# lab4d-org/lab4d

Hardware: AMD Instinct MI355X
Metric: rendered rays/sec (fwd+bwd) at 512² × 128 samples; PSNR vs ref (higher is better)
Workload: dtype bf16

## Files before the change

include/lab4d_skin.h:

```cpp
#ifndef LAB4D_SKIN_H
#define LAB4D_SKIN_H

int lab4d_bone_coords_forward(const float* xyz, const float* art_r, const float* art_d, const float* gauss, int S,
                              int spf, int M, int B, float* xyz_bone, void* stream);
int lab4d_bone_coords_backward(const float* xyz, const float* art_r, const float* art_d, const float* gauss,
                               const float* g_bone, int S, int spf, int M, int B, float* g_xyz, float* g_art_r,
                               float* g_art_d, float* g_gauss, void* stream);

int lab4d_bone_coords_backward_gram(const float* xyz, const float* art_r, const float* gauss, const float* g_bone, int S, int spf, int M, int B,
                                    float* g_xyz, float* G, void* stream);

int lab4d_bone_params_from_gram(const float* art_r, const float* art_d, const float* gauss, const float* G, int M, int B,
                                float* g_art_r, float* g_art_d, float* g_gauss, void* stream);

int lab4d_skin_blend_forward(const float* xyz, const float* art_r, const float* art_d, const float* gauss,
                             const float* delta_raw, const float* se3_r, const float* se3_d, int S, int spf, int M, int B,
                             float* out, float* entropy, float* dskin, float* work, void* stream);
int lab4d_skin_blend_backward(const float* xyz, const float* art_r, const float* art_d, const float* gauss,
                              const float* delta_raw, const float* se3_r, const float* se3_d, const float* g_out,
                              const float* g_ent, const float* g_dskin, int S, int spf, int M, int B, float* g_xyz,
                              float* g_raw, float* g_se3, float* g_art_r, float* g_art_d, float* g_gauss, float* work,
                              void* stream);
int lab4d_skin_blend_backward_acc(const float* xyz, const float* art_r, const float* art_d, const float* gauss,
                                  const float* delta_raw, const float* se3_r, const float* se3_d, const float* g_out,
                                  const float* g_ent, const float* g_dskin, int S, int spf, int M, int B, float* g_xyz,
                                  float* g_raw, float* g_se3, float* g_art_r, float* g_art_d, float* g_gauss, float* work,
                                  int accumulate, void* stream);

long long lab4d_skin_blend_backward_workspace_floats(int S, int spf, int M, int B, int has_g_se3);

int lab4d_gauss_density_forward(const float* xyz, const float* centres, int B, const float* ibeta, int S, float* out,
                                int* best, void* stream);
int lab4d_gauss_density_backward(const float* xyz, const float* centres, int B, const float* ibeta, const int* best,
                                 const float* g, int S, float* g_xyz, float* g_centres, float* g_ibeta, void* stream);

int lab4d_gram_per_frame(const float* A, int CA, const float* Bm, int CB, int S, int spf, int M, float* out, void* stream);

int lab4d_bone_affine(const float* art_r, const float* art_d, const float* gauss, int M, int B, float* aff, void* stream);

#endif
```

lab4d_amd/csrc/skinning.hip:

```cpp
#include "common.hpp"

namespace lab4d {

struct V3 { float x, y, z; };
__device__ __forceinline__ V3 operator+(V3 a, V3 b) { return {a.x + b.x, a.y + b.y, a.z + b.z}; }
__device__ __forceinline__ V3 operator-(V3 a, V3 b) { return {a.x - b.x, a.y - b.y, a.z - b.z}; }
__device__ __forceinline__ V3 operator*(V3 a, float s) { return {a.x * s, a.y * s, a.z * s}; }
__device__ __forceinline__ float dot(V3 a, V3 b) { return a.x * b.x + a.y * b.y + a.z * b.z; }
__device__ __forceinline__ V3 cross(V3 a, V3 b) { return {a.y * b.z - a.z * b.y, a.z * b.x - a.x * b.z, a.x * b.y - a.y * b.x}; }
__device__ __forceinline__ V3 ldv3(const float* p) { return {p[0], p[1], p[2]}; }
__device__ __forceinline__ void stv3(float* p, V3 v) { p[0] = v.x; p[1] = v.y; p[2] = v.z; }

__device__ __forceinline__ V3 qrot(float w, V3 v, V3 p) { return p * (w * w - dot(v, v)) + v * (2.f * dot(v, p)) + cross(v, p) * (2.f * w); }
__device__ __forceinline__ V3 qrot_t(float w, V3 v, V3 g) { return g * (w * w - dot(v, v)) + v * (2.f * dot(v, g)) - cross(v, g) * (2.f * w); }
__device__ __forceinline__ void qrot_gq(float w, V3 v, V3 p, V3 g, float& gw, V3& gv) {
  const float gp = dot(g, p), gvv = dot(g, v), vp = dot(v, p);
  gw = 2.f * w * gp + 2.f * dot(g, cross(v, p));
  gv = v * (-2.f * gp) + p * (2.f * gvv) + g * (2.f * vp) + cross(p, g) * (2.f * w);
}


template <int C>
struct RowTile {
  static constexpr int CP = C | 1;
// ... 490 lines not shown
        const float gskin = bl.p[b_] * (gp[b_] - pg) + ge * (bl.p[b_] - (b_ == bl.anchor ? 1.f : 0.f));
        const float gsk = -2.f * gskin;
        const Aff A = ld_aff(affm + 12 * b_);
        const V3 c = bone_coord(A, x);
        const float u0 = gsk * c.x, u1 = gsk * c.y, u2 = gsk * c.z;
        gx = gx + V3{A.r0.x * u0 + A.r1.x * u1 + A.r2.x * u2, A.r0.y * u0 + A.r1.y * u1 + A.r2.y * u2, A.r0.z * u0 + A.r1.z * u1 + A.r2.z * u2};
      }
      if (accumulate) gx = gx + ldv3(g_xyz + s * 3);
      stv3(g_xyz + s * 3, gx);
      if (!FUSE) {
        float* xx = work + S * (2 * B + 8) + s * 10;
        xx[0] = x.x * x.x; xx[1] = x.x * x.y; xx[2] = x.x * x.z; xx[3] = x.x;
        xx[4] = x.y * x.y; xx[5] = x.y * x.z; xx[6] = x.y;
        xx[7] = x.z * x.z; xx[8] = x.z; xx[9] = 1.f;
      }
    }
    __syncthreads();
    if (active) {
#pragma unroll
      for (int b_ = 0; b_ < B; ++b_) row[b_] = bl.p[b_] * bl.sg[b_];
    }
    __syncthreads();
    if (FUSE) gram(n, 8, 0);
    else { T::store(work, s0, n, tile); __syncthreads(); }
    if (active) {
#pragma unroll
      for (int b_ = 0; b_ < B; ++b_) {
        const float gskin = bl.p[b_] * (gp[b_] - pg) + ge * (bl.p[b_] - (b_ == bl.anchor ? 1.f : 0.f));
        row[b_] = -2.f * gskin;
      }
      if (FUSE) {
        float* xx = aux + threadIdx.x * AUXW;
        xx[0] = x.x * x.x; xx[1] = x.x * x.y; xx[2] = x.x * x.z; xx[3] = x.x;
        xx[4] = x.y * x.y; xx[5] = x.y * x.z; xx[6] = x.y;
        xx[7] = x.z * x.z; xx[8] = x.z; xx[9] = 1.f;
      }
    }
    __syncthreads();
    if (FUSE) gram(n, 10, B * 8);
    else { T::store(work + S * (B + 8), s0, n, tile); __syncthreads(); }
    if (active) {
#pragma unroll
      for (int b_ = 0; b_ < B; ++b_) {
        const float gskin = bl.p[b_] * (gp[b_] - pg) + ge * (bl.p[b_] - (b_ == bl.anchor ? 1.f : 0.f));
        const float gdelta = -gskin + gds * bl.dl[b_];
        row[b_] = ((rawpos >> b_) & 1u) ? 0.1f * gdelta : 0.f;
      }
    }
    __syncthreads();
    T::store(g_raw, s0, n, tile, accumulate);
    __syncthreads();
  }
  if (FUSE && cur_m >= 0) flush(cur_m);
}

__global__ void __launch_bounds__(64) k_bone_gram_from_moments(const float* __restrict__ ar, const float* __restrict__ ad,
                                                                const float* __restrict__ gauss, const float* __restrict__ Q, int M, int B,
                                                                float* __restrict__ G) {
  const int i = blockIdx.x * blockDim.x + threadIdx.x;
  if (i >= M * B) return;
  const int b = i % B;
  const float* r = ar + (size_t)i * 4;
  const float* d = ad + (size_t)i * 4;
  const float w = r[0], dw = d[0];
  const V3 v = ldv3(r + 1), dv = ldv3(d + 1), gs = ldv3(gauss + 3 * b);
  const V3 e0 = {1.f, 0.f, 0.f}, e1 = {0.f, 1.f, 0.f}, e2 = {0.f, 0.f, 1.f};
  const V3 t = (v * dw - dv * w + cross(v, dv)) * 2.f;
  const V3 c0 = qrot(w, v * -1.f, e0), c1 = qrot(w, v * -1.f, e1), c2 = qrot(w, v * -1.f, e2);
  const float A[3][4] = {{c0.x, c1.x, c2.x, t.x}, {c0.y, c1.y, c2.y, t.y}, {c0.z, c1.z, c2.z, t.z}};
  const float* q = Q + (size_t)i * 10;
  const float Qm[4][4] = {{q[0], q[1], q[2], q[3]}, {q[1], q[4], q[5], q[6]}, {q[2], q[5], q[7], q[8]}, {q[3], q[6], q[8], q[9]}};
  const float ig[3] = {1.f / gs.x, 1.f / gs.y, 1.f / gs.z};
  float* o = G + (size_t)i * 12;
#pragma unroll
  for (int k = 0; k < 3; ++k)
#pragma unroll
    for (int j = 0; j < 4; ++j) o[4 * k + j] = ig[k] * (A[k][0] * Qm[0][j] + A[k][1] * Qm[1][j] + A[k][2] * Qm[2][j] + A[k][3] * Qm[3][j]);
}

__global__ void __launch_bounds__(640) k_gram_pf(const float* __restrict__ A, int CA, const float* __restrict__ Bm, int CB, long S, int spf,
                                                  int chunk, float* __restrict__ out) {
  constexpr int TS = 128;
  extern __shared__ float sm[];
  float* sa = sm;
  float* sb = sm + TS * CA;
  const int m = blockIdx.y;
  const long f0 = (long)m * spf, f1 = min(S, f0 + spf);
  const long c0 = f0 + (long)blockIdx.x * chunk, c1 = min(f1, c0 + chunk);
  if (c0 >= c1) return;
  const int t = threadIdx.x;
  const int i = t / CB, j = t - i * CB;
  const bool active = t < CA * CB;
  float acc = 0.f;
  for (long s0 = c0; s0 < c1; s0 += TS) {
    const int n = (int)min((long)TS, c1 - s0);
    for (int e = t; e < n * CA; e += blockDim.x) sa[e] = A[s0 * CA + e];
    for (int e = t; e < n * CB; e += blockDim.x) sb[e] = Bm[s0 * CB + e];
    __syncthreads();
    if (active)
      for (int k = 0; k < n; ++k) acc += sa[k * CA + i] * sb[k * CB + j];
    __syncthreads();
  }
  if (active) atomicAdd(out + ((size_t)m * CA + i) * CB + j, acc);
}

template <int CB>
// ... 140 lines not shown
                                         const float* sr, const float* sd, const float* g_out, const float* g_ent, const float* g_dskin, int S,
                                         int spf, int M, int B, float* g_xyz, float* g_raw, float* g_se3, float* g_art_r, float* g_art_d,
                                         float* g_gauss, float* work, void* stream) {
  return lab4d_skin_blend_backward_acc(xyz, art_r, art_d, gauss, raw, sr, sd, g_out, g_ent, g_dskin, S, spf, M, B, g_xyz, g_raw, g_se3, g_art_r, g_art_d,
                                       g_gauss, work, 0, stream);
}
extern "C" int lab4d_skin_blend_backward_acc(const float* xyz, const float* art_r, const float* art_d, const float* gauss, const float* raw,
                                             const float* sr, const float* sd, const float* g_out, const float* g_ent, const float* g_dskin, int S,
                                             int spf, int M, int B, float* g_xyz, float* g_raw, float* g_se3, float* g_art_r, float* g_art_d,
                                             float* g_gauss, float* work, int accumulate, void* stream) {
  LAB4D_REQUIRE(xyz && art_r && art_d && gauss && raw && sr && sd && g_out && g_xyz && g_raw && work, "skin_blend_backward: null pointer");
  LAB4D_REQUIRE(spf > 0 && (long)M * spf >= S, "skin_blend_backward: M*spf < S");
  SKIN_REQUIRE_BONES(B);
  if (S == 0) return LAB4D_OK;
  hipStream_t st = (hipStream_t)stream;
  float* aff = work;
  float* Q = work + (size_t)M * B * 12;
  float* G = Q + (size_t)M * B * 10;
  float* ws = G + (size_t)M * B * 12;
  const bool fused = blend_bwd_fused(spf, g_se3 != nullptr);
  const bool params = g_art_r || g_art_d || g_gauss;
  hipLaunchKernelGGL(k_bone_affine, dim3(div_up(M * B, 64)), dim3(64), 0, st, art_r, art_d, gauss, M, B, aff);
  if (fused || params)
    if (int e = zero_async(Q, (size_t)M * B * 10 * sizeof(float), st)) return e;
  if (fused) {
    const int grid = grid_1d(S, 256, 2048);
#define BLEND_BWD(UNI_, FUSE_, GRID_)                                                                                                              \
  do {                                                                                                                                              \
    if (accumulate) { SKIN_DISPATCH(B, hipLaunchKernelGGL((k_blend_bwd<NB, UNI_, FUSE_, true>), dim3(GRID_), dim3(256), 0, st, xyz, aff, raw, sr, sd, g_out, \
                                                          g_ent, g_dskin, (long)S, spf, g_xyz, g_raw, ws, g_se3, Q)); }                              \
    else { SKIN_DISPATCH(B, hipLaunchKernelGGL((k_blend_bwd<NB, UNI_, FUSE_, false>), dim3(GRID_), dim3(256), 0, st, xyz, aff, raw, sr, sd, g_out,       \
                                               g_ent, g_dskin, (long)S, spf, g_xyz, g_raw, ws, g_se3, Q)); }                                         \
  } while (0)
    BLEND_BWD(true, true, grid);
  } else if (spf % 256 == 0) {
    BLEND_BWD(true, false, grid_1d(S, 256, 8192));
  } else {
    BLEND_BWD(false, false, grid_1d(S, 256, 8192));
  }
#undef BLEND_BWD
  if (int e = check_launch("skin_blend_backward")) return e;
  if (g_se3 && !fused)
    if (int e = lab4d_gram_per_frame(ws, B, ws + (size_t)S * B, 8, S, spf, M, g_se3, stream)) return e;
  if (params) {
    if (!fused)
      if (int e = lab4d_gram_per_frame(ws + (size_t)S * (B + 8), B, ws + (size_t)S * (2 * B + 8), 10, S, spf, M, Q, stream)) return e;
    hipLaunchKernelGGL(k_bone_gram_from_moments, dim3(div_up(M * B, 64)), dim3(64), 0, st, art_r, art_d, gauss, Q, M, B, G);
    if (int e = check_launch("bone_gram_from_moments")) return e;
    return lab4d_bone_params_from_gram(art_r, art_d, gauss, G, M, B, g_art_r, g_art_d, g_gauss, stream);
  }
  return LAB4D_OK;
}

namespace lab4d {
__global__ void __launch_bounds__(256) k_gauss_density_fwd(const float* __restrict__ xyz, const float* __restrict__ centres, int B,
                                                            const float* __restrict__ ibeta_p, long S, float* __restrict__ out, int* __restrict__ best) {
  const float ibeta = *ibeta_p;
  for (long s = (long)blockIdx.x * blockDim.x + threadIdx.x; s < S; s += (long)gridDim.x * blockDim.x) {
    const V3 x = ldv3(xyz + s * 3);
    float dmin = INFINITY;
    int bi = 0;
    for (int b = 0; b < B; ++b) {
      const V3 d = x - ldv3(centres + 3 * b);
      const float d2 = dot(d, d);
      if (d2 < dmin) { dmin = d2; bi = b; }
    }
    out[s] = expf(-0.5f * (dmin / (0.01f * 0.01f))) * ibeta;
    if (best) best[s] = bi;
  }
}
__global__ void __launch_bounds__(256) k_gauss_density_bwd(const float* __restrict__ xyz, const float* __restrict__ centres, int B,
                                                            const float* __restrict__ ibeta_p, const int* __restrict__ best, const float* __restrict__ g, long S,
                                                            float* __restrict__ g_xyz, float* __restrict__ g_centres, float* __restrict__ g_ibeta) {
  extern __shared__ float acc[];
  const float ibeta = *ibeta_p;
  for (int i = threadIdx.x; i < 3 * B + 1; i += blockDim.x) acc[i] = 0.f;
  __syncthreads();
  for (long s = (long)blockIdx.x * blockDim.x + threadIdx.x; s < S; s += (long)gridDim.x * blockDim.x) {
    const int b = best[s];
    const V3 d = ldv3(xyz + s * 3) - ldv3(centres + 3 * b);
    const float e = expf(-0.5f * (dot(d, d) / (0.01f * 0.01f)));
    const float gs = g[s];
    const V3 gx = d * (-gs * e * ibeta / (0.01f * 0.01f));
    if (g_xyz) stv3(g_xyz + s * 3, gx);
    atomicAdd(&acc[3 * b + 0], -gx.x); atomicAdd(&acc[3 * b + 1], -gx.y); atomicAdd(&acc[3 * b + 2], -gx.z);
    atomicAdd(&acc[3 * B], gs * e);
  }
  __syncthreads();
  for (int i = threadIdx.x; i < 3 * B; i += blockDim.x) if (acc[i] != 0.f) atomicAdd(g_centres + i, acc[i]);
  if (threadIdx.x == 0 && g_ibeta) atomicAdd(g_ibeta, acc[3 * B]);
}
}

extern "C" int lab4d_gauss_density_forward(const float* xyz, const float* centres, int B, const float* ibeta, int S, float* out, int* best, void* stream) {
  LAB4D_REQUIRE(xyz && centres && out && ibeta, "gauss_density_forward: null pointer");
  if (S == 0) return LAB4D_OK;
  hipLaunchKernelGGL(lab4d::k_gauss_density_fwd, dim3(grid_1d(S, 256, 8192)), dim3(256), 0, (hipStream_t)stream, xyz, centres, B, ibeta, (long)S, out, best);
  return check_launch("gauss_density_forward");
}
extern "C" int lab4d_gauss_density_backward(const float* xyz, const float* centres, int B, const float* ibeta, const int* best, const float* g, int S,
                                            float* g_xyz, float* g_centres, float* g_ibeta, void* stream) {
  LAB4D_REQUIRE(xyz && centres && ibeta && best && g && g_centres, "gauss_density_backward: null pointer");
  LAB4D_REQUIRE(B <= 64, "gauss_density_backward: B too large");
  if (S == 0) return LAB4D_OK;
  const int grid = grid_1d(S, 256, 1024);
  hipLaunchKernelGGL(lab4d::k_gauss_density_bwd, dim3(grid), dim3(256), (3 * B + 1) * sizeof(float), (hipStream_t)stream, xyz, centres, B, ibeta, best, g,
// ... 20 lines not shown
```

lab4d_amd/warping.py:

```python
import os

import torch
from torch.autograd import Function
from torch.autograd.function import once_differentiable

from . import _lib, mlp
from . import quat_utils as Q


def _blend_bwd_work(S, spf, M, B, device):
    n = int(_lib.lib().lab4d_skin_blend_backward_workspace_floats(S, spf, M, B, 1))
    return torch.empty(n, device=device), n == M * B * 34


FUSE_BONE_COORDS = os.environ.get("LAB4D_FUSE_BONE", "1") != "0"


class BoneCoords(Function):

    @staticmethod
    def forward(ctx, xyz, art_r, art_d, gauss, spf):
        xyz, art_r, art_d, gauss = xyz.contiguous(), art_r.contiguous(), art_d.contiguous(), gauss.contiguous()
        _lib.require_device(xyz, art_r, art_d, gauss)
        S, (M, B) = xyz.shape[0], art_r.shape[:2]
        out = torch.empty(S, 3 * B, device=xyz.device)
        with _lib.timed("k_bone_fwd", (0.0, 4.0 * S * (3 + 3 * B))):
            _lib.call("bone_coords_forward", xyz, art_r, art_d, gauss, S, spf, M, B, out)
        ctx.save_for_backward(xyz, art_r, art_d, gauss)
        ctx.spf = spf
        return out

    @staticmethod
    @once_differentiable
    def backward(ctx, g):
        return (*bone_coords_backward(ctx.saved_tensors, ctx.spf, ctx.needs_input_grad[1:4], g), None)


def bone_coords_backward(saved, spf, need, g):
    xyz, art_r, art_d, gauss = saved
    need_r, need_d, need_g = need
    S, (M, B) = xyz.shape[0], art_r.shape[:2]
    g = g.contiguous()
    gx = torch.empty_like(xyz)
    if any(need) and spf % 256 == 0 and os.environ.get("LAB4D_BONE_FUSE", "1") != "0":
        G = torch.empty(M, 3 * B, 4, device=xyz.device)
        with _lib.timed("k_bone_bwd_x+gram", (2.0 * S * 3 * B * 4, 4.0 * S * (3 + 3 + 3 * B))):
            _lib.call("bone_coords_backward_gram", xyz, art_r, gauss, g, S, spf, M, B, gx, G)
    else:
        with _lib.timed("k_bone_bwd_x", (0.0, 4.0 * S * (3 + 3 * B))):
            _lib.call("bone_coords_backward", xyz, art_r, art_d, gauss, g, S, spf, M, B, gx, None, None, None)
        if not any(need):
            return gx, None, None, None
# ... 78 lines not shown
    def forward(ctx, net, prec, spf, xyz, tab, *params):
        want = mlp.Wants(x=any(ctx.needs_input_grad), params=ctx.needs_input_grad[SkinChainA.N_LEAD:])
        out, _, ctx.chain = mlp.chain_forward(net, prec, spf, xyz.contiguous(), (), params, want, aff=tab.detach().contiguous())
        return out

    @staticmethod
    @once_differentiable
    def backward(ctx, d_out):
        d_x, _, _, _, g_params = mlp.chain_backward(ctx.chain, d_out)
        return (None, None, None, d_x, ctx.chain.g_aff, *g_params)


SKIN_AFFINE = os.environ.get("LAB4D_SKIN_AFFINE", "1") != "0"


class SkinBlend(Function):

    @staticmethod
    def forward(ctx, xyz, raw, art_r, art_d, gauss, se3_r, se3_d, spf):
        xyz, raw, art_r, art_d, gauss, se3_r, se3_d = [t.contiguous() for t in (xyz, raw, art_r, art_d, gauss, se3_r, se3_d)]
        _lib.require_device(xyz, raw, art_r, art_d, gauss, se3_r, se3_d)
        S, (M, B) = xyz.shape[0], se3_r.shape[:2]
        out = torch.empty(S, 3, device=xyz.device)
        ent = torch.empty(S, 1, device=xyz.device)
        dsk = torch.empty(S, 1, device=xyz.device)
        work = torch.empty(M * B * 12, device=xyz.device)
        with _lib.timed("k_blend_fwd", (0.0, 4.0 * S * (3 + B + 3 + 2))):
            _lib.call("skin_blend_forward", xyz, art_r, art_d, gauss, raw, se3_r, se3_d, S, spf, M, B, out, ent, dsk, work)
        ctx.save_for_backward(xyz, raw, art_r, art_d, gauss, se3_r, se3_d)
        ctx.spf = spf
        return out, ent, dsk

    @staticmethod
    @once_differentiable
    def backward(ctx, g_out, g_ent, g_dsk):
        xyz, raw, art_r, art_d, gauss, se3_r, se3_d = ctx.saved_tensors
        S, (M, B) = xyz.shape[0], se3_r.shape[:2]
        g_out = g_out.contiguous()
        g_ent = g_ent.contiguous() if g_ent is not None else None
        g_dsk = g_dsk.contiguous() if g_dsk is not None else None
        gx, gr = torch.empty_like(xyz), torch.empty_like(raw)
        gse3 = torch.zeros(M, B, 8, device=xyz.device)
        need_p = any(ctx.needs_input_grad[2:5])
        gar = torch.empty_like(art_r) if need_p else None
        gad = torch.empty_like(art_d) if need_p else None
        gg = torch.zeros_like(gauss) if need_p else None
        work, fused = _blend_bwd_work(S, ctx.spf, M, B, xyz.device)
        with _lib.timed("k_blend_bwd+gram", (0.0, 4.0 * S * ((3 + B + 3 + 2) + (3 + B) + (0 if fused else 2 * (2 * B + 18))))):
            _lib.call("skin_blend_backward", xyz, art_r, art_d, gauss, raw, se3_r, se3_d, g_out, g_ent, g_dsk, S, ctx.spf, M, B, gx, gr, gse3, gar, gad, gg,
                      work)
        return gx, gr, gar, gad, gg, gse3[..., :4].contiguous(), gse3[..., 4:].contiguous(), None


class SkinBlendMulti(Function):

    @staticmethod
    def forward(ctx, xyz, raw, art_r, art_d, gauss, spf, *se3s):
        xyz, raw, art_r, art_d, gauss = [t.contiguous() for t in (xyz, raw, art_r, art_d, gauss)]
        se3s = [t.contiguous() for t in se3s]
        _lib.require_device(xyz, raw, art_r, art_d, gauss, *se3s)
        S, (M, B) = xyz.shape[0], art_r.shape[:2]
        outs = []
        for i in range(0, len(se3s), 2):
            out = torch.empty(S, 3, device=xyz.device)
            ent = torch.empty(S, 1, device=xyz.device)
            dsk = torch.empty(S, 1, device=xyz.device)
            work = torch.empty(M * B * 12, device=xyz.device)
            with _lib.timed("k_blend_fwd", (0.0, 4.0 * S * (3 + B + 3 + 2))):
                _lib.call("skin_blend_forward", xyz, art_r, art_d, gauss, raw, se3s[i], se3s[i + 1], S, spf, M, B, out, ent, dsk, work)
            outs += [out, ent, dsk]
        ctx.save_for_backward(xyz, raw, art_r, art_d, gauss, *se3s)
        ctx.spf = spf
        return tuple(outs)

    @staticmethod
    @once_differentiable
    def backward(ctx, *grads):
        xyz, raw, art_r, art_d, gauss, *se3s = ctx.saved_tensors
        S, (M, B) = xyz.shape[0], art_r.shape[:2]
        gx, gr = torch.empty_like(xyz), torch.empty_like(raw)
        need_p = any(ctx.needs_input_grad[2:5])
        work0, fused = _blend_bwd_work(S, ctx.spf, M, B, xyz.device)
        gar = gad = gg = None
        gse3s = []
        first = True
        for i in range(0, len(se3s), 2):
            g_out, g_ent, g_dsk = grads[3 * (i // 2):3 * (i // 2) + 3]
            if g_out is None and g_ent is None and g_dsk is None:
                gse3s += [None, None]
                continue
            g_out = torch.zeros_like(xyz) if g_out is None else g_out.contiguous()
            g_ent = g_ent.contiguous() if g_ent is not None else None
            g_dsk = g_dsk.contiguous() if g_dsk is not None else None
            gse3 = torch.zeros(M, B, 8, device=xyz.device)
            par = torch.empty_like(art_r) if need_p else None
            pad = torch.empty_like(art_d) if need_p else None
            pg = torch.zeros_like(gauss) if need_p else None
            work = work0 if first else _blend_bwd_work(S, ctx.spf, M, B, xyz.device)[0]
            with _lib.timed("k_blend_bwd+gram", (0.0, 4.0 * S * ((3 + B + 3 + 2) + (3 + B) * (1 if first else 2) + (0 if fused else 2 * (2 * B + 18))))):
                _lib.call("skin_blend_backward_acc", xyz, art_r, art_d, gauss, raw, se3s[i], se3s[i + 1], g_out, g_ent, g_dsk, S, ctx.spf, M, B, gx, gr, gse3,
                          par, pad, pg, work, 0 if first else 1)
            first = False
            if need_p:
                gar, gad, gg = (par, pad, pg) if gar is None else (gar + par, gad + pad, gg + pg)
            gse3s += [gse3[..., :4].contiguous(), gse3[..., 4:].contiguous()]
        if first:
            return (None,) * (6 + len(se3s))
        return (gx, gr, gar, gad, gg, None) + tuple(gse3s)


def get_gauss(P):
    lg = P["warp.skinning_model.log_gauss"]
    symm = P.get("warp.skinning_model.symm_idx")
    if symm is not None:
        lg = (lg[symm] + lg) / 2
    return lg.exp()


def _spf(shape):
    spf = 1
    for d in shape[1:-1]:
        spf *= d
    return spf


def skin_cond(t_embed, code, M):
    return torch.cat([t_embed.expand(M, -1), code], -1)


def skin_logits(P, x, art, t_embed, code, M, spf, prec, pre=None):
    gauss = pre["gauss"] if pre is not None else get_gauss(P)
    B = art[0].shape[1]
    net = mlp.skin_net_for(B)
    d, bd = mlp.describe(net), mlp.bindings(net, "")
    if SKIN_AFFINE and FUSE_BONE_COORDS:
        tab = pre.get("tab") if pre is not None else None
        if tab is None:
            pf = pre["pf"] if pre is not None else mlp.pf_bias_of(net, 0, P[bd[0].wname], skin_cond(t_embed, code, M))
            tab = skin_affine_table(P, art, gauss, pf, B)
        net_a = mlp.skin_net_for(B, affine=True)
        bda = mlp.bindings(net_a, "")
        params = []
        for l in range(mlp.describe(net_a).n_layers):
            params += [P[bda[l].wname], P[bda[l].bname]]
        return SkinChainA.apply(net_a, prec, spf, x, tab, *params), gauss
    pf = pre["pf"] if pre is not None else mlp.pf_bias_of(net, 0, P[bd[0].wname], skin_cond(t_embed, code, M))
    params = []
    for l in range(d.n_layers):
        params += [P[bd[l].wname], P[bd[l].bname]]
    if not FUSE_BONE_COORDS:
        bone = BoneCoords.apply(x, art[0], art[1], gauss, spf)
        return mlp.MlpChain.apply(net, prec, spf, bone, None, None, -1, 1, None, None, pf, *params), gauss
    return SkinChain.apply(net, prec, spf, x, art[0], art[1], gauss, 1, pf, *params), gauss


def skinning_warp(P, xyz, t_articulation, rest_articulation, t_embed, code, backward, prec=mlp.PREC_F32, pre=None):
    shape = xyz.shape
    M, spf = shape[0], _spf(shape)
    if pre is not None:
        se3 = pre["se3"]
        art = t_articulation if backward else rest_articulation
    elif backward:
        se3 = Q.dual_quaternion_mul(rest_articulation, Q.dual_quaternion_inverse(t_articulation))
        art = t_articulation
    else:
        se3 = Q.dual_quaternion_mul(t_articulation, Q.dual_quaternion_inverse(rest_articulation))
        art = rest_articulation
    x = xyz.reshape(-1, 3)
    raw, gauss = skin_logits(P, x, art, t_embed, code, M, spf, prec, pre)
    out, ent, dsk = SkinBlend.apply(x, raw, art[0], art[1], gauss, se3[0], se3[1], spf)
    return out.view(shape), {"skin_entropy": ent.view(shape[:-1] + (1,)), "delta_skin": dsk.view(shape[:-1] + (1,))}


def skinning_warp_forward_multi(P, xyz, t_articulations, rest_articulation, t_embed_mean, code, prec=mlp.PREC_F32, pre=None):
    shape = xyz.shape
    M, spf = shape[0], _spf(shape)
    x = xyz.reshape(-1, 3)
    raw, gauss = skin_logits(P, x, rest_articulation, t_embed_mean, code, M, spf, prec, pre)
    rest_inv = None if pre is not None else Q.dual_quaternion_inverse(rest_articulation)
    se3s = [pre["se3s"][i] if pre is not None else Q.dual_quaternion_mul(t_art, rest_inv) for i, t_art in enumerate(t_articulations)]
    flat = SkinBlendMulti.apply(x, raw, rest_articulation[0], rest_articulation[1], gauss, spf, *[t for se3 in se3s for t in se3])
    outs = []
    for i in range(len(se3s)):
        out, ent, dsk = flat[3 * i:3 * i + 3]
        outs.append((out.view(shape), {"skin_entropy": ent.view(shape[:-1] + (1,)), "delta_skin": dsk.view(shape[:-1] + (1,))}))
    return outs


def dense_warp(P, xyz, t_embed, code, backward, prec=mlp.PREC_F32, prefix="warp.post_warp.", net=mlp.NET_DENSE):
    shape = xyz.shape
    spf = 1
    for d in shape[1:-1]:
        spf *= d
    which = "backward_map." if backward else "forward_map."
    cond = torch.cat([t_embed, code], -1)
    conds = {0: cond, 4: cond} if net == mlp.NET_DENSE6 else {0: cond}
    motion = mlp.run_chain(net, prec, P, xyz.reshape(-1, 3), spf, conds=conds, prefix=prefix + which)
    return xyz + 0.1 * motion.view(shape)


def composed_warp(P, xyz, t_articulation, rest_articulation, t_embed, code, backward, prec=mlp.PREC_F32, dense=None):
    if not backward and dense is not None:
        xyz = dense_warp(P, xyz, dense["t_embed"], dense["code_fw"], False, prec)
    out, aux = skinning_warp(P, xyz, t_articulation, rest_articulation, t_embed, code, backward, prec)
    if backward and dense is not None:
        out = dense_warp(P, out, dense["t_embed"], dense["code_bw"], True, prec)
    return out, aux
```

Before: 765,400.

## Fuse two-target skin blending into single forward and backward kernels

Adds multi-target blend kernels that compute the skinning weights once per point and apply them to both target SE3 sets in one pass, in both forward and backward. The backward kernel also fuses the per-frame Gram reductions for both targets plus the bone moments, avoiding repeated launches and repeated reads of xyz and raw logits. The Python wrapper now shares the entropy and delta-skin outputs across targets and dispatches to the fused path by default when the shape matches. The fused kernels are larger and use more shared memory and registers, which may reduce occupancy.

New measurement: 775,500, median of 6. +1.3%, better.

```diff
diff --git a/include/lab4d_skin.h b/include/lab4d_skin.h
--- a/include/lab4d_skin.h
+++ b/include/lab4d_skin.h
@@ -29,6 +29,14 @@
 
 long long lab4d_skin_blend_backward_workspace_floats(int S, int spf, int M, int B, int has_g_se3);
 
+int lab4d_skin_blend_forward_multi(const float* xyz, const float* art_r, const float* art_d, const float* gauss, const float* delta_raw, int T,
+                                   const float* const* se3_r, const float* const* se3_d, int S, int spf, int M, int B, float* const* out,
+                                   float* entropy, float* dskin, float* work, void* stream);
+int lab4d_skin_blend_backward_multi(const float* xyz, const float* art_r, const float* art_d, const float* gauss, const float* delta_raw, int T,
+                                    const float* const* se3_r, const float* const* se3_d, const float* const* g_out, const float* g_ent,
+                                    const float* g_dskin, int S, int spf, int M, int B, float* g_xyz, float* g_raw, float* const* g_se3,
+                                    float* g_art_r, float* g_art_d, float* g_gauss, float* work, void* stream);
+
 int lab4d_gauss_density_forward(const float* xyz, const float* centres, int B, const float* ibeta, int S, float* out,
                                 int* best, void* stream);
 int lab4d_gauss_density_backward(const float* xyz, const float* centres, int B, const float* ibeta, const int* best,
diff --git a/lab4d_amd/csrc/skinning.hip b/lab4d_amd/csrc/skinning.hip
--- a/lab4d_amd/csrc/skinning.hip
+++ b/lab4d_amd/csrc/skinning.hip
@@ -566,6 +566,270 @@
     __syncthreads();
   }
   if (FUSE && cur_m >= 0) flush(cur_m);
+}
+
+constexpr int BLEND_GROUP = 5;
+template <int B>
+struct SkinWeights {
+  float p[B];
+  float dl[B];
+  int anchor;
+  float lse_minus_max;
+};
+template <int B>
+__device__ __forceinline__ void skin_weights(V3 x, const float* __restrict__ affm, const float* __restrict__ raw, SkinWeights<B>& o) {
+  float skin[B];
+  float mx = -INFINITY;
+  int am = 0;
+#pragma unroll
+  for (int b = 0; b < B; ++b) {
+    const V3 c = bone_coord(ld_aff(affm + 12 * b), x);
+    const float dlt = fmaxf(raw[b], 0.f) * 0.1f;
+    o.dl[b] = dlt;
+    skin[b] = -(dot(c, c) + dlt);
+    if (skin[b] > mx) { mx = skin[b]; am = b; }
+  }
+  float sum = 0.f;
+#pragma unroll
+  for (int b = 0; b < B; ++b) { o.p[b] = expf(skin[b] - mx); sum += o.p[b]; }
+  const float isum = 1.f / sum;
+  o.anchor = am;
+  o.lse_minus_max = logf(sum);
+#pragma unroll
+  for (int b = 0; b < B; ++b) o.p[b] *= isum;
+}
+template <int B>
+__device__ __forceinline__ unsigned blend_target(const SkinWeights<B>& w, const float* __restrict__ sr, const float* __restrict__ sd, float (&rw)[4],
+                                                 float (&dw4)[4], float& inv) {
+  const int am = w.anchor;
+  const float a0 = sr[4 * am], a1 = sr[4 * am + 1], a2 = sr[4 * am + 2], a3 = sr[4 * am + 3];
+  unsigned neg = 0;
+#pragma unroll
+  for (int k = 0; k < 4; ++k) { rw[k] = 0.f; dw4[k] = 0.f; }
+#pragma unroll
+  for (int b = 0; b < B; ++b) {
+    if (b % BLEND_GROUP == 0) __builtin_amdgcn_sched_barrier(0);
+    const float* r = sr + 4 * b;
+    const float* d = sd + 4 * b;
+    const bool pos = (a0 * r[0] + a1 * r[1] + a2 * r[2] + a3 * r[3]) > 0.f;
+    neg |= (pos ? 0u : 1u) << b;
+    const float c = pos ? w.p[b] : -w.p[b];
+#pragma unroll
+    for (int k = 0; k < 4; ++k) { rw[k] += c * r[k]; dw4[k] += c * d[k]; }
+  }
+  __builtin_amdgcn_sched_barrier(0);
+  inv = 1.f / sqrtf(rw[0] * rw[0] + rw[1] * rw[1] + rw[2] * rw[2] + rw[3] * rw[3]);
+  return neg;
+}
+
+template <typename P>
+__device__ __forceinline__ P pick(int t, P a0, P a1) { return t == 0 ? a0 : a1; }
+
+template <int B, int T>
+__global__ void __launch_bounds__(256) k_blend_fwd_multi(const float* __restrict__ xyz, const float* __restrict__ aff, const float* __restrict__ raw,
+                                                          const float* __restrict__ sr0, const float* __restrict__ sd0, const float* __restrict__ sr1,
+                                                          const float* __restrict__ sd1, long S, int spf, float* __restrict__ out0,
+                                                          float* __restrict__ out1, float* __restrict__ ent, float* __restrict__ dskin) {
+  static_assert(T == 2, "the per-target pointer parameters are written out for two targets");
+  using R = RowTile<B>;
+  __shared__ float tile[R::FLOATS];
+  for (long s0 = (long)blockIdx.x * 256; s0 < S; s0 += (long)gridDim.x * 256) {
+    const long rem = S - s0;
+    const int n = (int)(rem < 256 ? rem : 256);
+    R::load(raw, s0, n, tile);
+    __syncthreads();
+    if ((int)threadIdx.x < n) {
+      const long s = s0 + threadIdx.x;
+      const int m = __builtin_amdgcn_readfirstlane(frame_of(s0, spf));
+      const V3 x = ldv3(xyz + s * 3);
+      SkinWeights<B> w;
+      skin_weights<B>(x, aff + (size_t)m * B * 12, tile + threadIdx.x * R::CP, w);
+#pragma unroll
+      for (int t = 0; t < T; ++t) {
+        float rw[4], dw4[4], i;
+        blend_target<B>(w, pick(t, sr0, sr1) + (size_t)m * B * 4, pick(t, sd0, sd1) + (size_t)m * B * 4, rw, dw4, i);
+        const V3 y = dq_apply(rw[0] * i, V3{rw[1], rw[2], rw[3]} * i, dw4[0] * i, V3{dw4[1], dw4[2], dw4[3]} * i, x);
+        stv3(pick(t, out0, out1) + s * 3, y);
+      }
+      if (ent) ent[s] = w.lse_minus_max;
+      if (dskin) {
+        float q = 0.f;
+#pragma unroll
+        for (int b = 0; b < B; ++b) q += w.dl[b] * w.dl[b];
+        dskin[s] = q / (float)B;
+      }
+    }
+    __syncthreads();
+  }
+}
+
+template <int B, int T>
+__global__ void __launch_bounds__(256, 2) k_blend_bwd_multi(const float* __restrict__ xyz, const float* __restrict__ aff, const float* __restrict__ raw,
+                                                             const float* __restrict__ sr0, const float* __restrict__ sd0, const float* __restrict__ sr1,
+                                                             const float* __restrict__ sd1, const float* __restrict__ g_out0,
+                                                             const float* __restrict__ g_out1, const float* __restrict__ g_ent,
+                                                             const float* __restrict__ g_dskin, long S, int spf, float* __restrict__ g_xyz,
+                                                             float* __restrict__ g_raw, float* __restrict__ g_se3_0, float* __restrict__ g_se3_1,
+                                                             float* __restrict__ Qm) {
+  static_assert(T == 2, "the per-target pointer parameters are written out for two targets");
+  using R = RowTile<B>;
+  __shared__ float tile[R::FLOATS];
+  constexpr int AUXW = 12;
+  constexpr int SLICES = 256 / B;
+  constexpr int NSE3 = T * B * 8;
+  static_assert(R::FLOATS >= SLICES * B * 10, "the tile doubles as the slice-reduction scratch");
+  __shared__ __attribute__((aligned(16))) float aux[256 * AUXW];
+  __shared__ float lacc[NSE3 + B * 10];
+  __shared__ float keep[R::FLOATS];
+  int cur_m = -1;
+  for (int e = threadIdx.x; e < NSE3 + B * 10; e += 256) lacc[e] = 0.f;
+  auto flush = [&](int m) {
+    for (int e = threadIdx.x; e < NSE3 + B * 10; e += 256) {
+      const float v = lacc[e];
+      if (v != 0.f) {
+        if (e < NSE3) { const int t = e / (B * 8); atomicAdd(pick(t, g_se3_0, g_se3_1) + (size_t)m * B * 8 + (e - t * B * 8), v); }
+        else atomicAdd(Qm + (size_t)m * B * 10 + (e - NSE3), v);
+      }
+      lacc[e] = 0.f;
+    }
+  };
+  auto gram = [&](int n, int ncol, int off) {
+    const int t = threadIdx.x, sl = t / B, i = t - sl * B;
+    const bool act = sl < SLICES;
+    float acc[10];
+#pragma unroll
+    for (int j = 0; j < 10; ++j) acc[j] = 0.f;
+    if (act)
+      for (int k = sl; k < n; k += SLICES) {
+        const float a = tile[k * R::CP + i];
+        const float4 b0 = *reinterpret_cast<const float4*>(aux + k * AUXW), b1 = *reinterpret_cast<const float4*>(aux + k * AUXW + 4);
+        acc[0] += a * b0.x; acc[1] += a * b0.y; acc[2] += a * b0.z; acc[3] += a * b0.w;
+        acc[4] += a * b1.x; acc[5] += a * b1.y; acc[6] += a * b1.z; acc[7] += a * b1.w;
+        if (ncol == 10) {
+          const float2 b2 = *reinterpret_cast<const float2*>(aux + k * AUXW + 8);
+          acc[8] += a * b2.x; acc[9] += a * b2.y;
+        }
+      }
+    __syncthreads();
+    if (act)
+      for (int j = 0; j < ncol; ++j) tile[(sl * B + i) * ncol + j] = acc[j];
+    __syncthreads();
+    for (int e = t; e < B * ncol; e += 256) {
+      float v = 0.f;
+#pragma unroll
+      for (int q = 0; q < SLICES; ++q) v += tile[q * B * ncol + e];
+      lacc[off + e] += v;
+    }
+    __syncthreads();
+  };
+  for (long s0 = (long)blockIdx.x * 256; s0 < S; s0 += (long)gridDim.x * 256) {
+    const long rem = S - s0;
+    const int n = (int)(rem < 256 ? rem : 256);
+    const bool active = (int)threadIdx.x < n;
+    const long s = s0 + threadIdx.x;
+    float* row = tile + threadIdx.x * R::CP;
+    const int m = __builtin_amdgcn_readfirstlane(frame_of(s0, spf));
+    if (m != cur_m) {
+      if (cur_m >= 0) { __syncthreads(); flush(cur_m); }
+      cur_m = m;
+    }
+    R::load(raw, s0, n, keep);
+    __syncthreads();
+    const float* rawrow = keep + threadIdx.x * R::CP;
+    SkinWeights<B> w;
+    float gp[B];
+    const float* affm = aff + (size_t)m * B * 12;
+    V3 x = {0, 0, 0}, gx = {0, 0, 0};
+    if (active) {
+      x = ldv3(xyz + s * 3);
+      skin_weights<B>(x, affm, rawrow, w);
+#pragma unroll
+      for (int b_ = 0; b_ < B; ++b_) gp[b_] = 0.f;
+    }
+#pragma unroll
+    for (int t = 0; t < T; ++t) {
+      const float* srm = pick(t, sr0, sr1) + (size_t)m * B * 4;
+      const float* sdm = pick(t, sd0, sd1) + (size_t)m * B * 4;
+      int zero = 0;
+      asm volatile("" : "+v"(zero));
+      const int again = m * B * 4 + __builtin_amdgcn_readfirstlane(zero);
+      if (active) {
+        const V3 g = ldv3(pick(t, g_out0, g_out1) + s * 3);
+        float rw[4], dw4[4], i;
+        const unsigned neg = blend_target<B>(w, srm, sdm, rw, dw4, i);
+        const float qw = rw[0] * i, dw = dw4[0] * i;
+        const V3 v = V3{rw[1], rw[2], rw[3]} * i, dv = V3{dw4[1], dw4[2], dw4[3]} * i;
+        gx = gx + qrot_t(qw, v, g);
+        float gqw; V3 gqv;
+        qrot_gq(qw, v, x, g, gqw, gqv);
+        const float gn_w = gqw + 2.f * dot(dv, g);
+        const V3 gn_v = gqv + g * (-2.f * dw) + cross(dv, g) * 2.f;
+        const float gd_w = -2.f * dot(v, g);
+        const V3 gd_v = g * (2.f * qw) + cross(g, v) * 2.f;
+        const float qg = qw * gn_w + dot(v, gn_v);
+        const float dg = dw * gd_w + dot(dv, gd_v);
+        float grw[4], gdw[4];
+        grw[0] = i * (gn_w - qw * qg) - qw * i * dg;
+        grw[1] = i * (gn_v.x - v.x * qg) - v.x * i * dg;
+        grw[2] = i * (gn_v.y - v.y * qg) - v.y * i * dg;
+        grw[3] = i * (gn_v.z - v.z * qg) - v.z * i * dg;
+        gdw[0] = i * gd_w; gdw[1] = i * gd_v.x; gdw[2] = i * gd_v.y; gdw[3] = i * gd_v.z;
+        float4* wg = reinterpret_cast<float4*>(aux + threadIdx.x * AUXW);
+        wg[0] = make_float4(grw[0], grw[1], grw[2], grw[3]);
+        wg[1] = make_float4(gdw[0], gdw[1], gdw[2], gdw[3]);
+#pragma unroll
+        for (int b_ = 0; b_ < B; ++b_) {
+          if (b_ % BLEND_GROUP == 0) __builtin_amdgcn_sched_barrier(0);
+          const float* r = pick(t, sr0, sr1) + again + 4 * b_;
+          const float* d = pick(t, sd0, sd1) + again + 4 * b_;
+          const float gpb = r[0] * grw[0] + r[1] * grw[1] + r[2] * grw[2] + r[3] * grw[3] + d[0] * gdw[0] + d[1] * gdw[1] + d[2] * gdw[2] + d[3] * gdw[3];
+          const bool ng = (neg >> b_) & 1u;
+          gp[b_] += ng ? -gpb : gpb;
+          row[b_] = ng ? -w.p[b_] : w.p[b_];
+        }
+        __builtin_amdgcn_sched_barrier(0);
+      }
+      __syncthreads();
+      gram(n, 8, t * B * 8);
+    }
+    float pg = 0.f, ge = 0.f, gds = 0.f;
+    if (active) {
+#pragma unroll
+      for (int b_ = 0; b_ < B; ++b_) pg += w.p[b_] * gp[b_];
+      ge = g_ent ? g_ent[s] : 0.f;
+      gds = g_dskin ? g_dskin[s] * (2.f / (float)B) : 0.f;
+#pragma unroll
+      for (int b_ = 0; b_ < B; ++b_) {
+        const float gskin = w.p[b_] * (gp[b_] - pg) + ge * (w.p[b_] - (b_ == w.anchor ? 1.f : 0.f));
+        const float gsk = -2.f * gskin;
+        const Aff A = ld_aff(affm + 12 * b_);
+        const V3 c = bone_coord(A, x);
+        const float u0 = gsk * c.x, u1 = gsk * c.y, u2 = gsk * c.z;
+        gx = gx + V3{A.r0.x * u0 + A.r1.x * u1 + A.r2.x * u2, A.r0.y * u0 + A.r1.y * u1 + A.r2.y * u2, A.r0.z * u0 + A.r1.z * u1 + A.r2.z * u2};
+        row[b_] = gsk;
+      }
+      stv3(g_xyz + s * 3, gx);
+      float* xx = aux + threadIdx.x * AUXW;
+      xx[0] = x.x * x.x; xx[1] = x.x * x.y; xx[2] = x.x * x.z; xx[3] = x.x;
+      xx[4] = x.y * x.y; xx[5] = x.y * x.z; xx[6] = x.y;
+      xx[7] = x.z * x.z; xx[8] = x.z; xx[9] = 1.f;
+    }
+    __syncthreads();
+    gram(n, 10, NSE3);
+    if (active) {
+#pragma unroll
+      for (int b_ = 0; b_ < B; ++b_) {
+        const float gskin = w.p[b_] * (gp[b_] - pg) + ge * (w.p[b_] - (b_ == w.anchor ? 1.f : 0.f));
+        const float rb = rawrow[b_];
+        const float gdelta = -gskin + gds * (fmaxf(rb, 0.f) * 0.1f);
+        row[b_] = rb > 0.f ? 0.1f * gdelta : 0.f;
+      }
+    }
+    __syncthreads();
+    R::store(g_raw, s0, n, tile);
+    __syncthreads();
+  }
+  if (cur_m >= 0) flush(cur_m);
 }
 
 __global__ void __launch_bounds__(64) k_bone_gram_from_moments(const float* __restrict__ ar, const float* __restrict__ ad,
@@ -812,6 +1076,54 @@
   return LAB4D_OK;
 }
 
+#define SKIN_MULTI_T 2
+static bool blend_multi_shape(int T, int spf, int B) { return T == SKIN_MULTI_T && spf > 0 && spf % 256 == 0 && (B == 25 || B == 18); }
+#define SKIN_MULTI_REQUIRE(WHAT, T, spf, B)                                                                                                     \
+  LAB4D_REQUIRE(blend_multi_shape(T, spf, B), WHAT ": instantiated for T = 2 targets, spf %% 256 == 0 and B = 25 or 18; got T=%d spf=%d B=%d " \
+                "(use the single-target entry per target)", T, spf, B)
+
+extern "C" int lab4d_skin_blend_forward_multi(const float* xyz, const float* art_r, const float* art_d, const float* gauss, const float* raw, int T,
+                                              const float* const* sr, const float* const* sd, int S, int spf, int M, int B, float* const* out,
+                                              float* ent, float* dskin, float* work, void* stream) {
+  LAB4D_REQUIRE(xyz && art_r && art_d && gauss && raw && sr && sd && out && work, "skin_blend_forward_multi: null pointer");
+  SKIN_MULTI_REQUIRE("skin_blend_forward_multi", T, spf, B);
+  LAB4D_REQUIRE((long)M * spf >= S, "skin_blend_forward_multi: M*spf < S");
+  for (int t = 0; t < SKIN_MULTI_T; ++t) LAB4D_REQUIRE(sr[t] && sd[t] && out[t], "skin_blend_forward_multi: null pointer (target %d)", t);
+  if (S == 0) return LAB4D_OK;
+  hipStream_t st = (hipStream_t)stream;
+  hipLaunchKernelGGL(k_bone_affine, dim3(div_up(M * B, 64)), dim3(64), 0, st, art_r, art_d, gauss, M, B, work);
+  SKIN_DISPATCH(B, hipLaunchKernelGGL((k_blend_fwd_multi<NB, SKIN_MULTI_T>), dim3(grid_1d(S, 256, 8192)), dim3(256), 0, st, xyz, work, raw, sr[0], sd[0], sr[1], sd[1], (long)S, spf, out[0], out[1], ent, dskin));
+  return check_launch("skin_blend_forward_multi");
+}
+
+extern "C" int lab4d_skin_blend_backward_multi(const float* xyz, const float* art_r, const float* art_d, const float* gauss, const float* raw, int T,
+                                               const float* const* sr, const float* const* sd, const float* const* g_out, const float* g_ent,
+                                               const float* g_dskin, int S, int spf, int M, int B, float* g_xyz, float* g_raw, float* const* g_se3,
+                                               float* g_art_r, float* g_art_d, float* g_gauss, float* work, void* stream) {
+  LAB4D_REQUIRE(xyz && art_r && art_d && gauss && raw && sr && sd && g_out && g_xyz && g_raw && g_se3 && work, "skin_blend_backward_multi: null pointer");
+  SKIN_MULTI_REQUIRE("skin_blend_backward_multi", T, spf, B);
+  LAB4D_REQUIRE(blend_bwd_fused(spf, true), "skin_blend_backward_multi: needs the fused adjoint (LAB4D_BLEND_FUSE=0 is set)");
+  LAB4D_REQUIRE((long)M * spf >= S, "skin_blend_backward_multi: M*spf < S");
+  for (int t = 0; t < SKIN_MULTI_T; ++t) LAB4D_REQUIRE(sr[t] && sd[t] && g_out[t] && g_se3[t], "skin_blend_backward_multi: null pointer (target %d)", t);
+  if (S == 0) return LAB4D_OK;
+  hipStream_t st = (hipStream_t)stream;
+  float* aff = work;
+  float* Q = work + (size_t)M * B * 12;
+  float* G = Q + (size_t)M * B * 10;
+  const bool params = g_art_r || g_art_d || g_gauss;
+  hipLaunchKernelGGL(k_bone_affine, dim3(div_up(M * B, 64)), dim3(64), 0, st, art_r, art_d, gauss, M, B, aff);
+  if (int e = zero_async(Q, (size_t)M * B * 10 * sizeof(float), st)) return e;
+  const int grid = grid_1d(S, 256, 2048);
+  SKIN_DISPATCH(B, hipLaunchKernelGGL((k_blend_bwd_multi<NB, SKIN_MULTI_T>), dim3(grid), dim3(256), 0, st, xyz, aff, raw, sr[0], sd[0], sr[1], sd[1], g_out[0], g_out[1], g_ent, g_dskin, (long)S, spf, g_xyz, g_raw, g_se3[0], g_se3[1], Q));
+  if (int e = check_launch("skin_blend_backward_multi")) return e;
+  if (params) {
+    hipLaunchKernelGGL(k_bone_gram_from_moments, dim3(div_up(M * B, 64)), dim3(64), 0, st, art_r, art_d, gauss, Q, M, B, G);
+    if (int e = check_launch("bone_gram_from_moments")) return e;
+    return lab4d_bone_params_from_gram(art_r, art_d, gauss, G, M, B, g_art_r, g_art_d, g_gauss, stream);
+  }
+  return LAB4D_OK;
+}
+
 namespace lab4d {
 __global__ void __launch_bounds__(256) k_gauss_density_fwd(const float* __restrict__ xyz, const float* __restrict__ centres, int B,
                                                             const float* __restrict__ ibeta_p, long S, float* __restrict__ out, int* __restrict__ best) {
diff --git a/lab4d_amd/warping.py b/lab4d_amd/warping.py
--- a/lab4d_amd/warping.py
+++ b/lab4d_amd/warping.py
@@ -1,3 +1,4 @@
+import ctypes
 import os
 
 import torch
@@ -182,6 +183,24 @@
         return gx, gr, gar, gad, gg, gse3[..., :4].contiguous(), gse3[..., 4:].contiguous(), None
 
 
+SKIN_BLEND_MULTI = os.environ.get("LAB4D_SKIN_BLEND_MULTI", "1") != "0"
+
+
+def _blend_multi_shape(spf, B, T):
+    return SKIN_BLEND_MULTI and T == 2 and spf % 256 == 0 and B in (18, 25)
+
+
+def _blend_multi_work(S, spf, M, B, T, device):
+    if not _blend_multi_shape(spf, B, T):
+        return None
+    work, fused = _blend_bwd_work(S, spf, M, B, device)
+    return work if fused else None
+
+
+def _pointers(tensors):
+    return (ctypes.c_void_p * len(tensors))(*[t.data_ptr() for t in tensors])
+
+
 class SkinBlendMulti(Function):
 
     @staticmethod
@@ -190,52 +209,64 @@
         se3s = [t.contiguous() for t in se3s]
         _lib.require_device(xyz, raw, art_r, art_d, gauss, *se3s)
         S, (M, B) = xyz.shape[0], art_r.shape[:2]
-        outs = []
-        for i in range(0, len(se3s), 2):
-            out = torch.empty(S, 3, device=xyz.device)
-            ent = torch.empty(S, 1, device=xyz.device)
-            dsk = torch.empty(S, 1, device=xyz.device)
-            work = torch.empty(M * B * 12, device=xyz.device)
-            with _lib.timed("k_blend_fwd", (0.0, 4.0 * S * (3 + B + 3 + 2))):
-                _lib.call("skin_blend_forward", xyz, art_r, art_d, gauss, raw, se3s[i], se3s[i + 1], S, spf, M, B, out, ent, dsk, work)
-            outs += [out, ent, dsk]
+        T = len(se3s) // 2
+        outs = [torch.empty(S, 3, device=xyz.device) for _ in range(T)]
+        ent = torch.empty(S, 1, device=xyz.device)
+        dsk = torch.empty(S, 1, device=xyz.device)
+        work = torch.empty(M * B * 12, device=xyz.device)
+        if _blend_multi_shape(spf, B, T):
+            with _lib.timed("k_blend_fwd_multi", (0.0, 4.0 * S * (3 + B + 3 * T + 2))):
+                _lib.call("skin_blend_forward_multi", xyz, art_r, art_d, gauss, raw, T, _pointers(se3s[0::2]), _pointers(se3s[1::2]), S, spf, M, B,
+                          _pointers(outs), ent, dsk, work)
+        else:
+            for i in range(T):
+                with _lib.timed("k_blend_fwd", (0.0, 4.0 * S * (3 + B + 3 + (2 if i == 0 else 0)))):
+                    _lib.call("skin_blend_forward", xyz, art_r, art_d, gauss, raw, se3s[2 * i], se3s[2 * i + 1], S, spf, M, B, outs[i],
+                              ent if i == 0 else None, dsk if i == 0 else None, work)
         ctx.save_for_backward(xyz, raw, art_r, art_d, gauss, *se3s)
         ctx.spf = spf
-        return tuple(outs)
+        return tuple(outs) + (ent, dsk)
 
     @staticmethod
     @once_differentiable
     def backward(ctx, *grads):
         xyz, raw, art_r, art_d, gauss, *se3s = ctx.saved_tensors
         S, (M, B) = xyz.shape[0], art_r.shape[:2]
+        T = len(se3s) // 2
+        g_outs, (g_ent, g_dsk) = list(grads[:T]), grads[T:]
+        if all(g is None for g in grads):
+            return (None,) * (6 + len(se3s))
+        g_ent = g_ent.contiguous() if g_ent is not None else None
+        g_dsk = g_dsk.contiguous() if g_dsk is not None else None
+        live = [i for i in range(T) if g_outs[i] is not None] or [0]
+        g_outs = [torch.zeros_like(xyz) if (g is None and i in live) else (g.contiguous() if g is not None else None) for i, g in enumerate(g_outs)]
         gx, gr = torch.empty_like(xyz), torch.empty_like(raw)
         need_p = any(ctx.needs_input_grad[2:5])
-        work0, fused = _blend_bwd_work(S, ctx.spf, M, B, xyz.device)
-        gar = gad = gg = None
+        gse3 = {i: torch.zeros(M, B, 8, device=xyz.device) for i in live}
+        work = _blend_multi_work(S, ctx.spf, M, B, T, xyz.device) if len(live) == T else None
+        if work is not None:
+            gar = torch.empty_like(art_r) if need_p else None
+            gad = torch.empty_like(art_d) if need_p else None
+            gg = torch.zeros_like(gauss) if need_p else None
+            with _lib.timed("k_blend_bwd_multi+gram", (0.0, 4.0 * S * ((3 + B + 3 * T + 2) + (3 + B)))):
+                _lib.call("skin_blend_backward_multi", xyz, art_r, art_d, gauss, raw, T, _pointers(se3s[0::2]), _pointers(se3s[1::2]), _pointers(g_outs),
+                          g_ent, g_dsk, S, ctx.spf, M, B, gx, gr, _pointers([gse3[i] for i in range(T)]), gar, gad, gg, work)
+        else:
+            gar = gad = gg = None
+            for k, i in enumerate(live):
+                first, last = k == 0, k == len(live) - 1
+                work, fused = _blend_bwd_work(S, ctx.spf, M, B, xyz.device)
+                par = torch.empty_like(art_r) if need_p else None
+                pad = torch.empty_like(art_d) if need_p else None
+                pg = torch.zeros_like(gauss) if need_p else None
+                with _lib.timed("k_blend_bwd+gram", (0.0, 4.0 * S * ((3 + B + 3 + 2) + (3 + B) * (1 if first else 2) + (0 if fused else 2 * (2 * B + 18))))):
+                    _lib.call("skin_blend_backward_acc", xyz, art_r, art_d, gauss, raw, se3s[2 * i], se3s[2 * i + 1], g_outs[i], g_ent if last else None,
+                              g_dsk if last else None, S, ctx.spf, M, B, gx, gr, gse3[i], par, pad, pg, work, 0 if first else 1)
+                if need_p:
+                    gar, gad, gg = (par, pad, pg) if gar is None else (gar + par, gad + pad, gg + pg)
         gse3s = []
-        first = True
-        for i in range(0, len(se3s), 2):
-            g_out, g_ent, g_dsk = grads[3 * (i // 2):3 * (i // 2) + 3]
-            if g_out is None and g_ent is None and g_dsk is None:
-                gse3s += [None, None]
-                continue
-            g_out = torch.zeros_like(xyz) if g_out is None else g_out.contiguous()
-            g_ent = g_ent.contiguous() if g_ent is not None else None
-            g_dsk = g_dsk.contiguous() if g_dsk is not None else None
-            gse3 = torch.zeros(M, B, 8, device=xyz.device)
-            par = torch.empty_like(art_r) if need_p else None
-            pad = torch.empty_like(art_d) if need_p else None
-            pg = torch.zeros_like(gauss) if need_p else None
-            work = work0 if first else _blend_bwd_work(S, ctx.spf, M, B, xyz.device)[0]
-            with _lib.timed("k_blend_bwd+gram", (0.0, 4.0 * S * ((3 + B + 3 + 2) + (3 + B) * (1 if first else 2) + (0 if fused else 2 * (2 * B + 18))))):
-                _lib.call("skin_blend_backward_acc", xyz, art_r, art_d, gauss, raw, se3s[i], se3s[i + 1], g_out, g_ent, g_dsk, S, ctx.spf, M, B, gx, gr, gse3,
-                          par, pad, pg, work, 0 if first else 1)
-            first = False
-            if need_p:
-                gar, gad, gg = (par, pad, pg) if gar is None else (gar + par, gad + pad, gg + pg)
-            gse3s += [gse3[..., :4].contiguous(), gse3[..., 4:].contiguous()]
-        if first:
-            return (None,) * (6 + len(se3s))
+        for i in range(T):
+            gse3s += [gse3[i][..., :4].contiguous(), gse3[i][..., 4:].contiguous()] if i in gse3 else [None, None]
         return (gx, gr, gar, gad, gg, None) + tuple(gse3s)
 
 
@@ -310,11 +341,8 @@
     rest_inv = None if pre is not None else Q.dual_quaternion_inverse(rest_articulation)
     se3s = [pre["se3s"][i] if pre is not None else Q.dual_quaternion_mul(t_art, rest_inv) for i, t_art in enumerate(t_articulations)]
     flat = SkinBlendMulti.apply(x, raw, rest_articulation[0], rest_articulation[1], gauss, spf, *[t for se3 in se3s for t in se3])
-    outs = []
-    for i in range(len(se3s)):
-        out, ent, dsk = flat[3 * i:3 * i + 3]
-        outs.append((out.view(shape), {"skin_entropy": ent.view(shape[:-1] + (1,)), "delta_skin": dsk.view(shape[:-1] + (1,))}))
-    return outs
+    ent, dsk = flat[len(se3s):]
+    return [(out.view(shape), {"skin_entropy": ent.view(shape[:-1] + (1,)), "delta_skin": dsk.view(shape[:-1] + (1,))}) for out in flat[:len(se3s)]]
 
 
 def dense_warp(P, xyz, t_embed, code, backward, prec=mlp.PREC_F32, prefix="warp.post_warp.", net=mlp.NET_DENSE):
```
